# dmlc/difacto

Hardware: AMD Instinct MI355X
Metric: examples/sec (FM SGD worker step, Criteo-shape, V_dim=64) (higher is better)
Workload: dtype f32

## Files before the change

difacto_amd/capi.py:

```python
import ctypes as C
import os

import numpy as np

_HERE = os.path.dirname(os.path.abspath(__file__))
LIB_PATH = os.environ.get("DIFACTO_HIP_LIB") or os.path.join(_HERE, "libdifacto_hip.so")

FEA_COUNT, WEIGHT, GRADIENT = 1, 2, 3
INIT_REFRAND, INIT_HASH = 0, 1
U64MAX = 2 ** 64 - 1

SYMBOLS = [
    "dfh_last_error", "dfh_updater_param_default", "dfh_ctx_create", "dfh_ctx_destroy", "dfh_ctx_sync",
    "dfh_ctx_stream", "dfh_ctx_device", "dfh_reverse_bytes", "dfh_encode_fea_grp_id", "dfh_table_create",
    "dfh_table_destroy", "dfh_table_size", "dfh_table_param", "dfh_table_bytes", "dfh_pull", "dfh_push",
    "dfh_table_export", "dfh_table_import", "dfh_fm_predict", "dfh_fm_calcgrad", "dfh_loss_evaluate",
    "dfh_auc_times_n", "dfh_batch_create", "dfh_batch_destroy", "dfh_batch_load_host", "dfh_batch_load_device",
    "dfh_localize", "dfh_batch_load_localized_host", "dfh_batch_get_localized", "dfh_batch_shape", "dfh_sgd_step",
    "dfh_batch_progress", "dfh_batch_get_pred", "dfh_row_stride", "dfh_shard_pull", "dfh_shard_push_count",
    "dfh_shard_push_grad", "dfh_batch_forward", "dfh_batch_backward", "dfh_batch_device_keys", "dfh_malloc",
    "dfh_free", "dfh_memcpy_h2d", "dfh_memcpy_d2h", "dfh_ctx_set_timing", "dfh_ctx_get_timing", "dfh_kernel_name",
    "dfh_table_warm_start", "dfh_ctx_set_pipeline", "dfh_batch_lookup", "dfh_localize_lookup", "dfh_rowbuf_create", "dfh_rowbuf_destroy", "dfh_rowbuf_load_host", "dfh_batch_gather_rows", "dfh_batch_set_option", "dfh_batch_key_ranges", "dfh_batch_attach_device",
    "dfh_batch_key_ranges_device", "dfh_shard_resolve", "dfh_shard_pull_resolved", "dfh_shard_push_count_resolved",
    "dfh_shard_push_grad_resolved", "dfh_table_check", "dfh_ctx_set_timing_mask", "dfh_table_save", "dfh_table_load", "dfh_shard_resolve_multi", "dfh_shard_push_count_multi",
    "dfh_shard_push_grad_multi", "dfh_shard_count_pull_multi", "dfh_shard_push_grad_listed", "dfh_shard_release", "dfh_ctx_set_option", "dfh_table_set_has_aux", "dfh_table_has_aux",
    "dfh_comm_unique_id", "dfh_comm_create_rccl", "dfh_comm_create_callback", "dfh_comm_destroy", "dfh_comm_rank", "dfh_comm_world",
    "dfh_comm_allreduce_sum", "dfh_shard_create", "dfh_shard_destroy", "dfh_shard_owned_range", "dfh_shard_step", "dfh_shard_prefetch_counts",
    "dfh_shard_pull_host", "dfh_shard_push_host", "dfh_comm_allgather", "dfh_shard_balanced_splits", "dfh_shard_set_exchange", "dfh_shard_set_timing", "dfh_shard_get_timing",
    "dfh_comm_stats", "dfh_comm_info", "dfh_comm_selfcheck", "dfh_comm_wire_probe", "dfh_table_capacity", "dfh_batch_prepare_rows", "dfh_rowbuf_load_host_slices",
    "dfh_rowbuf_set_labels", "dfh_batch_prepare_cached", "dfh_batch_get_rows",
    "dfh_batch_create_many", "dfh_shard_multi_words", "dfh_shard_reserve", "dfh_comm_create_loopback", "dfh_comm_loopback_feed", "dfh_comm_loopback_wire", "dfh_comm_loopback_wire_time",
    "dfh_vec_inner_multi", "dfh_vec_combine", "dfh_vec_line_step", "dfh_lbfgs_create", "dfh_lbfgs_destroy", "dfh_lbfgs_add_chunk",
    "dfh_lbfgs_init_model", "dfh_lbfgs_shape", "dfh_lbfgs_get_model", "dfh_lbfgs_set_weights", "dfh_lbfgs_calc_grad",
    "dfh_lbfgs_prepare_direction", "dfh_lbfgs_calc_direction", "dfh_lbfgs_line_search", "dfh_lbfgs_evaluate", "dfh_lbfgs_create_sharded",
    "dfh_lbfgs_owned_range", "dfh_lbfgs_set_model", "dfh_lbfgs_get_vector", "dfh_bcd_set_model",
    "dfh_bcd_create", "dfh_bcd_destroy", "dfh_bcd_add_chunk", "dfh_bcd_build", "dfh_bcd_shape", "dfh_bcd_block_info",
    "dfh_bcd_epoch", "dfh_bcd_step", "dfh_bcd_get_model", "dfh_bcd_get_pred", "dfh_batch_split_entries",
    "dfh_bcd_create_sharded",
    "dfh_textchunk_create", "dfh_textchunk_destroy", "dfh_textchunk_parse_criteo", "dfh_textchunk_rows", "dfh_textchunk_ids",
    "dfh_rowbuf_load_slices",
]
XCHG_COUNTS, XCHG_KEYS, XCHG_CNT, XCHG_ROWS, XCHG_GRADS, XCHG_OTHER = range(6)
SHARD_STAGES = ("counts", "L", "K", "R", "RW", "F", "G", "P")
K_COUNT = 8
K_LOCALIZE, K_LOOKUP, K_FORWARD, K_BACKWARD, K_PULL, K_PUSH, K_MISC, K_AUC = range(8)


class UpdaterParam(C.Structure):
    _fields_ = [("l1", C.c_float), ("l2", C.c_float), ("V_l2", C.c_float), ("lr", C.c_float),
                ("lr_beta", C.c_float), ("V_lr", C.c_float), ("V_lr_beta", C.c_float),
                ("V_init_scale", C.c_float), ("V_dim", C.c_int), ("V_threshold", C.c_int),
                ("seed", C.c_uint), ("init_mode", C.c_int)]


class Progress(C.Structure):
    _fields_ = [("loss", C.c_float), ("penalty", C.c_float), ("auc", C.c_float),
                ("nnz_w", C.c_float), ("nrows", C.c_float)]


class Slice(C.Structure):
# ... 40 lines not shown
    L.dfh_reverse_bytes.restype = u64
    L.dfh_reverse_bytes.argtypes = [u64]
    L.dfh_encode_fea_grp_id.restype = u64
    L.dfh_encode_fea_grp_id.argtypes = [u64, i32, i32]
    L.dfh_table_create.argtypes = [vp, PP(UpdaterParam), u64, PP(vp)]
    L.dfh_table_destroy.argtypes = [vp]
    L.dfh_table_size.argtypes = [vp, PP(u64)]
    L.dfh_table_param.argtypes = [vp, PP(UpdaterParam)]
    L.dfh_table_capacity.argtypes = [vp, PP(u64), PP(u64)]
    L.dfh_table_bytes.restype = u64
    L.dfh_table_bytes.argtypes = [vp]
    L.dfh_pull.argtypes = [vp, vp, sz, vp, PP(sz), vp, PP(sz)]
    L.dfh_push.argtypes = [vp, vp, sz, i32, vp, sz, vp, sz]
    L.dfh_table_export.argtypes = [vp, u64, vp, vp, vp, vp, PP(u64)]
    L.dfh_table_import.argtypes = [vp, u64, vp, vp, vp, vp]
    L.dfh_fm_predict.argtypes = [vp, i32, sz, vp, vp, vp, vp, sz, vp, vp, sz, vp]
    L.dfh_fm_calcgrad.argtypes = [vp, i32, sz, vp, vp, vp, vp, vp, sz, vp, vp, sz, vp, vp]
    L.dfh_loss_evaluate.argtypes = [vp, vp, vp, sz, PP(f32)]
    L.dfh_auc_times_n.argtypes = [vp, vp, vp, sz, PP(f32)]
    L.dfh_batch_create.argtypes = [vp, sz, sz, PP(vp)]
    L.dfh_batch_destroy.argtypes = [vp]
    L.dfh_batch_create_many.argtypes = [vp, i32, sz, sz, PP(vp)]
    L.dfh_batch_split_entries.argtypes = [vp, vp]
    L.dfh_batch_load_host.argtypes = [vp, sz, vp, vp, vp, vp]
    L.dfh_batch_load_device.argtypes = [vp, sz, sz, vp, vp, vp, vp]
    L.dfh_batch_attach_device.argtypes = [vp, sz, sz, vp, vp, vp, vp]
    L.dfh_localize.argtypes = [vp, u64]
    L.dfh_batch_load_localized_host.argtypes = [vp, sz, vp, vp, vp, vp, vp, vp, sz]
    L.dfh_batch_get_localized.argtypes = [vp, PP(sz), vp, vp, vp]
    L.dfh_batch_shape.argtypes = [vp, PP(sz), PP(sz), PP(sz)]
    L.dfh_sgd_step.argtypes = [vp, vp, i32, i32]
    L.dfh_batch_progress.argtypes = [vp, PP(Progress), i32]
    L.dfh_batch_get_pred.argtypes = [vp, vp]
    L.dfh_row_stride.restype = sz
    L.dfh_row_stride.argtypes = [i32]
    L.dfh_shard_pull.argtypes = [vp, vp, sz, vp]
    L.dfh_shard_push_count.argtypes = [vp, vp, sz, vp]
    L.dfh_shard_push_grad.argtypes = [vp, vp, sz, vp]
    L.dfh_batch_forward.argtypes = [vp, i32, vp]
    L.dfh_batch_backward.argtypes = [vp, i32, vp, vp]
    L.dfh_batch_device_keys.argtypes = [vp, PP(vp), PP(vp), PP(sz)]
    L.dfh_malloc.argtypes = [vp, sz, PP(vp)]
    L.dfh_free.argtypes = [vp, vp]
    L.dfh_memcpy_h2d.argtypes = [vp, vp, vp, sz]
    L.dfh_memcpy_d2h.argtypes = [vp, vp, vp, sz]
    L.dfh_table_warm_start.argtypes = [vp, vp, sz, f32, f32]
# ... 539 lines not shown
        lab = np.zeros(nrows, np.float32)
        _ck(lib().dfh_batch_get_rows(self.h, _p(off), _p(lab)))
        return off, lab

    def sgd_step(self, table, is_train=True, push_cnt=False):
        _ck(lib().dfh_sgd_step(table.h, self.h, 1 if is_train else 0, 1 if push_cnt else 0))

    def progress(self, reset=True):
        p = Progress()
        _ck(lib().dfh_batch_progress(self.h, C.byref(p), 1 if reset else 0))
        return p

    def pred(self):
        nrows, _, _ = self.shape(want_U=False)
        out = np.zeros(nrows, np.float32)
        _ck(lib().dfh_batch_get_pred(self.h, _p(out)))
        return out

    def split_entries(self):
        n = C.c_uint32(0)
        _ck(lib().dfh_batch_split_entries(self.h, C.byref(n)))
        return int(n.value)

    def forward(self, V_dim, d_rows):
        _ck(lib().dfh_batch_forward(self.h, V_dim, _dp(d_rows)))

    def backward(self, V_dim, d_rows, d_grads):
        _ck(lib().dfh_batch_backward(self.h, V_dim, _dp(d_rows), _dp(d_grads)))

    def key_ranges(self, nparts):
        out = np.zeros(nparts + 1, np.uint32)
        _ck(lib().dfh_batch_key_ranges(self.h, nparts, _p(out)))
        return out

    def device_keys(self):
        a, b, u = C.c_void_p(), C.c_void_p(), C.c_size_t(0)
        _ck(lib().dfh_batch_device_keys(self.h, C.byref(a), C.byref(b), C.byref(u)))
        return a.value, b.value, u.value

    def device_key_ptrs(self):
        a, b = C.c_void_p(), C.c_void_p()
        _ck(lib().dfh_batch_device_keys(self.h, C.byref(a), C.byref(b), None))
        return a.value, b.value

    def key_ranges_device(self, nparts, d_bounds, d_splits=None):
        _ck(lib().dfh_batch_key_ranges_device(self.h, nparts, _dp(d_splits), _dp(d_bounds)))
# ... 385 lines not shown
```

difacto_amd/csrc/dfh_api.hip:

```cpp
#include <algorithm>
#include <chrono>
#include <cstring>
#include <mutex>
#include <new>
#include <thread>

#include <hip/hip_ext.h>
#include <rocprim/rocprim.hpp>

#include "dfh_kernels.hip"
#include "dfh_localize.hip"
#include "dfh_update.hip"
#include "dfh_riders.hip"

using namespace dfh;

namespace dfh {
static thread_local std::string g_err;
void set_error(const std::string& msg) { g_err = msg; }
}

struct dfh_ctx {
  int device = 0;
  hipStream_t stream = nullptr;
// ... 2435 lines not shown
    v.bkeys = b->d_keys;
    v.bpos = b->d_bpos;
    v.skeys = b->d_skeys;
    v.spos = b->d_spos;
    v.first_key = b->d_first_key;
    v.last_key = b->d_last_key;
    v.nheads = b->d_nheads;
    v.lh = b->d_lh;
    EmitOut& o = b->loc_o;
    o.value = b->has_value ? b->d_value : (const float*)nullptr;
    o.feaids = b->d_feaids;
    o.col_ptr = b->d_col_ptr;
    o.index = b->d_index;
    o.s_row = b->d_s_row;
    o.s_val = b->d_s_val;
    o.d_U = b->d_U;
    o.sl.mid = b->d_mid;
    o.sl.mid_ent = b->d_mid_ent;
    o.sl.hot = b->d_hot;
    o.sl.hot_ent = b->d_hot_ent;
    o.sl.few = b->d_few;
    o.sl.few_ent = b->d_few_ent;
    v.split_n = b->d_U + 2;
    b->loc_big = big;
#ifndef DFH_LOC_GRID_CAP
#define DFH_LOC_GRID_CAP 1024
#endif
    b->loc_gsort = (unsigned)std::min<int>(P, big ? LOC_BIG_BUCKETS : DFH_LOC_GRID_CAP);
    if (cold && P > 1) {
      const uint32_t S = (uint32_t)P * LOC_OVERSAMPLE;
      const uint32_t nt = (S + 255) / 256;
      hipLaunchKernelGGL(k_ss_sample, dim3(nt), dim3(256), 0, s, v);
      hipLaunchKernelGGL(k_ss_rank, dim3(nt * nt), dim3(256), 0, s, v);
      hipLaunchKernelGGL(k_loc_splitters, dim3(nt), dim3(256), 0, s, v);
    }
    if (c->single_queue && !cold && !big && !probe) {
      b->pend_stage = 0;
      c->pend.push_back(b);
    } else {
      for (int st = 0; st < RID_STAGES; ++st) {
        launch_loc_stage(b, st, s, probe);
        if (st == RID_COUNT && b->loc_fuse_gather) {
          int rcg = gather_queued(b, s);
          b->loc_fuse_gather = false;
          if (rcg) return rcg;
        }
      }
    }
    b->spl_P = P;
    b->seg_nb = (uint32_t)P;
  } else {
    hipLaunchKernelGGL(k_rdx_keys, dim3(g), dim3(256), 0, s, b->d_raw, N, max_index, b->d_keys, b->d_pos);
    size_t tb = b->temp_bytes;
    DFH_HIP(rocprim::radix_sort_pairs(b->d_temp, tb, b->d_keys, b->d_skeys, b->d_pos, b->d_spos, (size_t)N, 0, 64, s));
    hipLaunchKernelGGL(k_rdx_heads, dim3(g), dim3(256), 0, s, b->d_skeys, N, b->d_head);
    tb = b->temp_bytes;
    DFH_HIP(rocprim::inclusive_scan(b->d_temp, tb, b->d_head, b->d_uid, (size_t)N, rocprim::plus<uint32_t>(), s));
    hipLaunchKernelGGL(k_rdx_emit, dim3(g), dim3(256), 0, s, b->d_skeys, b->d_spos, b->d_head, b->d_uid, N, (uint32_t)b->nrows,
                       b->d_offset, b->has_value ? b->d_value : (const float*)nullptr, b->d_feaids, b->d_col_ptr, b->d_index,
                       b->d_s_row, b->d_s_val, b->d_U);
    hipLaunchKernelGGL(k_seg_lists_reset, dim3(1), dim3(64), 0, s, b->d_mid, b->d_hot, b->d_few, b->d_U + 2);
    hipLaunchKernelGGL(k_seg_lists, dim3((unsigned)std::max<size_t>(1, std::min<size_t>((N + 1023) / 1024, 256))), dim3(1024), 0, s,
                       b->d_col_ptr, b->d_U, b->d_mid, b->d_hot, b->d_few, b->d_mid_ent, b->d_hot_ent, b->d_few_ent);
    b->seg_nb = 1;
    if (probe)
      hipLaunchKernelGGL(k_lookup, dim3(grid_for_threads(b->nnz, c)), dim3(256), 0, s, probe->v, b->d_feaids, b->d_U, 0u, b->d_urow,
                         (const float*)nullptr, b->d_col_ptr, 0, (uint32_t*)nullptr, 0, (uint2*)nullptr, AucFin{nullptr, 0u, nullptr});
  }
  delete tsp;
  DFH_HIP(hipGetLastError());
  b->localized = true;
  b->has_cnt = false;
  if (probe) b->looked_up = probe;
  return prep_end(b);
// ... 263 lines not shown
  }
  rc = step_math(t, b, is_train, push_cnt, kAllKeys, nullptr, x, [&](bool) -> int {
    if (is_train && refrand) DFH_HIP(hipMemsetAsync(b->d_need, 0, (size_t)Nb * 4, s));
    return DFH_OK;
  });
  if (rc) return rc;
  if (is_train && refrand) {
    rc = refrand_flush(t, b->d_feaids, b->d_U, Nb, b->d_urow, b->d_need, b->d_rank, b->d_total);
    if (rc) return rc;
  }
  return main_end(b);
}

int dfh_batch_split_entries(dfh_batch* b, uint32_t* n) {
  DFH_ARG(b && n, "dfh_batch_split_entries: NULL argument");
  dfh_ctx* c = b->ctx;
  DFH_HIP(hipSetDevice(c->device));
  if (b->pend_stage < RID_STAGES) {
    int rc = flush_pending(b);
    if (rc) return rc;
  }
  if (b->ready_pending) DFH_HIP(hipStreamWaitEvent(c->stream, b->ev_ready, 0));
  DFH_HIP(hipMemcpyAsync(n, b->d_U + 2 + b->split_last, sizeof(uint32_t), hipMemcpyDeviceToHost, c->stream));
  DFH_HIP(hipStreamSynchronize(c->stream));
  return DFH_OK;
}

int dfh_batch_forward(dfh_batch* b, int V_dim, const float* d_rows) {
  DFH_ARG(b && b->localized && d_rows, "dfh_batch_forward: bad argument");
  const int kp = (V_dim + 3) / 4 * 4;
  int rc = ensure_xv(b, kp);
  if (rc) return rc;
  b->nrows_seen += (float)b->nrows;
  rc = main_begin(b);
  if (rc) return rc;
  rc = launch_forward(b, packed_src(d_rows, V_dim), V_dim, kp);
  if (rc) return rc;
  return main_end(b);
}

int dfh_batch_backward(dfh_batch* b, int V_dim, const float* d_rows, float* d_grads) {
  DFH_ARG(b && b->localized && d_rows && d_grads, "dfh_batch_backward: bad argument");
  const int kp = (V_dim + 3) / 4 * 4;
  if (b->nnz == 0) return DFH_OK;
  TableView dummy{};
  int rc = launch_backward<false>(b, packed_src(d_rows, V_dim), dummy, d_grads, dfh_row_stride(V_dim), V_dim, kp, nullptr);
// ... 93 lines not shown
```

difacto_amd/csrc/dfh_localize.hip:

```cpp
#ifndef DFH_LOCALIZE_HIP_
#define DFH_LOCALIZE_HIP_
#include "dfh_internal.h"
#include "dfh_feed_layout.h"

namespace dfh {

constexpr int LOC_OVERSAMPLE = 8;
constexpr int LOC_MAX_BUCKETS = 1024;
constexpr int LOC_BIG_BUCKETS = 4096;
constexpr int LOC_AVG_BUCKET = 384;
constexpr int LOC_MIN_AVG = 48;
constexpr int LOC_MAX_AVG = 700;
constexpr int LOC_LDS_CAP = 1024;
#ifndef DFH_LOC_TILE_THREADS
#define DFH_LOC_TILE_THREADS 1024
#endif
constexpr int LOC_TILE_THREADS = DFH_LOC_TILE_THREADS;
constexpr int LOC_PER_THREAD = LOC_TILE / LOC_TILE_THREADS;
constexpr int LOC_SORT_THREADS = 256;
constexpr int LOC_EMIT_THREADS = 256;

struct LocView {
  const uint64_t* raw;
  uint32_t n;
// ... 3 lines not shown
  int ntiles;
  int force_global;
  int tb;
  uint32_t nrows;
  const uint32_t* offset;
  const uint32_t* rowid;
  uint64_t* smp_key;
  uint32_t* smp_pos;
  uint32_t* smp_rank;
  uint64_t* spl_key;
  uint32_t* spl_pos;
  uint32_t* packed;
  uint32_t* run_off;
  uint32_t* btotal;
  uint32_t* bstart;
  uint64_t* bkeys;
  uint32_t* bpos;
  uint64_t* skeys;
  uint32_t* spos;
  uint64_t* first_key;
  uint64_t* last_key;
  uint32_t* nheads;
  uint32_t* lh;
  uint32_t* split_n;
};

struct SegListsOut {
  uint2* mid;
  SegEnt* mid_ent;
  uint2* hot;
  SegEnt* hot_ent;
  uint2* few;
  SegEnt* few_ent;
};

__device__ __forceinline__ uint64_t make_key(uint64_t id, uint64_t max_index) {
  const uint64_t m = (max_index == ~0ULL) ? (id == ~0ULL ? 0ULL : id) : id % max_index;
  return reverse_bytes(m);
}

constexpr int LOC_XCDS = 8;

__device__ __forceinline__ bool comp_less(uint64_t ka, uint32_t pa, uint64_t kb, uint32_t pb) {
  return ka < kb || (ka == kb && pa < pb);
}

// ... 96 lines not shown
  const float* src_val[LOC_GATHER_SEGS];
  const uint32_t* h_rows;
  const uint32_t* h_off;
  const float* h_lab;
  const uint32_t* h_tile_row;
  uint64_t* dst_raw;
  float* dst_val;
  uint32_t* dst_off;
  float* dst_lab;
};
constexpr size_t loc_gather_smem() { return (size_t)(LOC_GATHER_ROWS + 1) * 4 + 4 + (size_t)LOC_GATHER_ROWS * 8; }
template <typename T>
__device__ __forceinline__ T loc_sel(const T (&a)[LOC_GATHER_SEGS], uint32_t sg) {
  T r = a[0];
#pragma unroll
  for (int x = 1; x < LOC_GATHER_SEGS; ++x) r = sg == (uint32_t)x ? a[x] : r;
  return r;
}

template <int MAXB>
constexpr size_t loc_count_smem() { return (size_t)MAXB * 16; }
template <int MAXB, int THREADS>
constexpr size_t loc_scatter_smem() { return (size_t)MAXB * 4 + (THREADS / 64) * 4; }
constexpr size_t loc_sort_smem() { return (size_t)LOC_LDS_CAP * 24 + 2 * (LOC_SORT_THREADS / 64) * 4; }
constexpr size_t loc_emit_smem() { return (2 * (LOC_EMIT_THREADS / 64) + 4) * 4; }

template <int MAXB, int THREADS, bool GATHER = false>
__device__ __forceinline__ void loc_count_block(const LocView& v, const uint32_t bid, const uint32_t nblk, char* smem,
                                                const GatherSrc* gp = nullptr) {
  constexpr int PER = LOC_TILE / THREADS;
  static_assert(PER * THREADS == LOC_TILE, "a tile is a whole number of elements per thread");
  uint64_t* sk = reinterpret_cast<uint64_t*>(smem);
  uint32_t* sp = reinterpret_cast<uint32_t*>(smem + (size_t)MAXB * 8);
  uint32_t* hist = sp + MAXB;
  const int P = v.P;
  for (int b = threadIdx.x; b < P; b += THREADS) {
    hist[b] = 0;
    sk[b] = b < P - 1 ? v.spl_key[b] : ~0ULL;
    sp[b] = b < P - 1 ? v.spl_pos[b] : ~0u;
  }
  const uint32_t base = bid * LOC_TILE;
  if (bid == 0 && threadIdx.x == 0 && v.split_n) *v.split_n = 0u;
  uint64_t key[PER];
  if (GATHER) {
    const GatherSrc& g = *gp;
    uint32_t* roff = reinterpret_cast<uint32_t*>(smem + loc_count_smem<MAXB>());
    uint64_t* rsrc = reinterpret_cast<uint64_t*>(roff + LOC_GATHER_ROWS + 2);
    const uint32_t row0 = g.h_tile_row[bid], row1 = g.h_tile_row[bid + 1];
    const uint32_t nr = min(row1, v.nrows - 1u) - row0 + 1u;
    for (uint32_t q = threadIdx.x; q <= nr; q += THREADS) roff[q] = g.h_off[row0 + q];
    for (uint32_t q = threadIdx.x; q < nr; q += THREADS) {
      const uint32_t r = row0 + q;
      uint32_t sg = 0;
#pragma unroll
      for (int x = 1; x < LOC_GATHER_SEGS; ++x) sg += (x < g.nseg && r >= g.seg_row0[x]) ? 1u : 0u;
      rsrc[q] = ((uint64_t)loc_sel(g.src_off, sg)[g.h_rows[r]] << 2) | sg;
    }
    __syncthreads();
#pragma unroll
    for (int e = 0; e < PER; ++e) {
      const uint32_t i = base + e * THREADS + threadIdx.x;
      key[e] = ~0ULL;
      if (i < v.n) {
        uint32_t lo = 0, hi = nr - 1u;
// ... 158 lines not shown

template <int MAXB>
__global__ void __launch_bounds__(LOC_TILE_THREADS) k_loc_scatter(LocView v) {
  __shared__ __attribute__((aligned(16))) char smem[loc_scatter_smem<MAXB, LOC_TILE_THREADS>()];
  loc_scatter_block<MAXB, LOC_TILE_THREADS>(v, blockIdx.x, smem);
}

template <int J>
__device__ __forceinline__ uint32_t loc_net_partner(uint32_t x) {
  static_assert(J == 1 || J == 2 || J == 4 || J == 8, "DPP reaches the partners inside a row of 16 lanes");
  if constexpr (J == 1) return (uint32_t)__builtin_amdgcn_mov_dpp((int)x, 0xB1, 0xf, 0xf, false);
  if constexpr (J == 2) return (uint32_t)__builtin_amdgcn_mov_dpp((int)x, 0x4E, 0xf, 0xf, false);
  if constexpr (J == 4) {
    const int y = __builtin_amdgcn_mov_dpp((int)x, 0x141, 0xf, 0xf, false);
    return (uint32_t)__builtin_amdgcn_mov_dpp(y, 0x1B, 0xf, 0xf, false);
  }
  return (uint32_t)__builtin_amdgcn_mov_dpp((int)x, 0x128, 0xf, 0xf, false);
}
constexpr uint64_t loc_net_keeps_max(int K, int J) {
  uint64_t m = 0;
  for (int i = 0; i < 64; ++i) m |= (uint64_t)(((i & J) != 0) != ((i & K) != 0)) << i;
  return m;
}
template <int K, int J>
__device__ __forceinline__ void loc_net_stage(uint32_t& klo, uint32_t& khi, uint32_t& tag) {
  uint32_t mlo, mhi;
  asm volatile("s_mov_b32 %0, %2\n\ts_mov_b32 %1, %3"
               : "=s"(mlo), "=s"(mhi)
               : "i"((int32_t)(uint32_t)loc_net_keeps_max(K, J)), "i"((int32_t)(uint32_t)(loc_net_keeps_max(K, J) >> 32)));
  const uint64_t mask = ((uint64_t)mhi << 32) | mlo;
  const bool keeps_max = __builtin_amdgcn_inverse_ballot_w64(mask);
  if constexpr (J >= 16) {
    uint32_t alo, ahi, at, blo, bhi, bt;
#define DFH_NET_SWAP(a, b, x)                                                                                       \
    {                                                                                                                 \
      const auto r = J == 16 ? __builtin_amdgcn_permlane16_swap(x, x, false, false) : __builtin_amdgcn_permlane32_swap(x, x, false, false); \
      a = r[0];                                                                                                       \
      b = r[1];                                                                                                       \
    }
    DFH_NET_SWAP(alo, blo, klo)
    DFH_NET_SWAP(ahi, bhi, khi)
    DFH_NET_SWAP(at, bt, tag)
#undef DFH_NET_SWAP
    const bool out_of_order = comp_less(((uint64_t)bhi << 32) | blo, bt, ((uint64_t)ahi << 32) | alo, at);
    const bool take_b = out_of_order != keeps_max;
    klo = take_b ? blo : alo;
    khi = take_b ? bhi : ahi;
    tag = take_b ? bt : at;
  } else {
    const uint32_t olo = loc_net_partner<J>(klo), ohi = loc_net_partner<J>(khi), ot = loc_net_partner<J>(tag);
    const bool partner_less = comp_less(((uint64_t)ohi << 32) | olo, ot, ((uint64_t)khi << 32) | klo, tag);
    const bool take = partner_less != keeps_max;
    klo = take ? olo : klo;
    khi = take ? ohi : khi;
    tag = take ? ot : tag;
  }
}
template <int K, int J>
__device__ __forceinline__ void loc_net_merge(uint32_t& klo, uint32_t& khi, uint32_t& tag) {
  loc_net_stage<K, J>(klo, khi, tag);
  if constexpr (J > 1) loc_net_merge<K, J / 2>(klo, khi, tag);
}
template <int K = 2>
__device__ __forceinline__ void loc_net_sort64(uint32_t& klo, uint32_t& khi, uint32_t& tag) {
  loc_net_merge<K, K / 2>(klo, khi, tag);
  if constexpr (K < 64) loc_net_sort64<K * 2>(klo, khi, tag);
}

__device__ __forceinline__ bool loc_sort_bucket_lds(const LocView& v, uint32_t beg, uint32_t n, uint64_t* ak, uint32_t* ap,
                                                    uint64_t* bk, uint32_t* bp) {
  const uint64_t* gk = v.bkeys + beg;
  const uint32_t* gp = v.bpos + beg;
  uint64_t* sk = bk;
  uint32_t* sp = bp;
  const uint32_t lane = threadIdx.x & 63;
  for (uint32_t c0 = (threadIdx.x >> 6) * 64; c0 < n; c0 += LOC_SORT_THREADS) {
    const uint32_t idx = c0 + lane;
    const bool valid = idx < n;
    const uint64_t mk = valid ? gk[idx] : ~0ULL;
    uint32_t klo = (uint32_t)mk, khi = (uint32_t)(mk >> 32);
    uint32_t mp = valid ? gp[idx] : ~0u;
    loc_net_sort64(klo, khi, mp);
    if (valid) {
      bk[idx] = ((uint64_t)khi << 32) | klo;
      bp[idx] = mp;
    }
  }
  __syncthreads();
  constexpr int E = LOC_LDS_CAP / LOC_SORT_THREADS;
  constexpr int G = 2;
  static_assert(E * LOC_SORT_THREADS == LOC_LDS_CAP && E % G == 0 && LOC_SORT_THREADS % 64 == 0,
                "a thread carries E elements of a full bucket, G at a time");
  uint64_t* dk = ak;
  uint32_t* dp = ap;
  uint32_t sh = 6;
  for (uint32_t L = 64; L < n; L <<= 1, ++sh) {
    for (int g = 0; g < E && g * LOC_SORT_THREADS < (int)n; g += G) {
      uint64_t mk[G];
      uint32_t mp[G], at[G], end[G];
#pragma unroll
      for (int e = 0; e < G; ++e) {
        const uint32_t idx = threadIdx.x + (g + e) * LOC_SORT_THREADS;
        const bool valid = idx < n;
        const uint32_t sib = ((idx >> sh) ^ 1u) << sh;
        mk[e] = valid ? sk[idx] : 0ULL;
// ... 1 lines not shown
        at[e] = min(sib, n);
        end[e] = valid ? min(sib + L, n) : at[e];
      }
      for (uint32_t step = L; step; step >>= 1) {
        uint64_t ok[G];
        uint32_t op[G];
#pragma unroll
        for (int e = 0; e < G; ++e) {
          const uint32_t q = at[e] + step <= end[e] ? at[e] + step - 1u : 0u;
          ok[e] = sk[q];
          op[e] = sp[q];
        }
#pragma unroll
        for (int e = 0; e < G; ++e)
          if (at[e] + step <= end[e] && comp_less(ok[e], op[e], mk[e], mp[e])) at[e] += step;
      }
#pragma unroll
      for (int e = 0; e < G; ++e) {
        const uint32_t idx = threadIdx.x + (g + e) * LOC_SORT_THREADS;
        if (idx < n) {
          const uint32_t dst = idx + at[e] - min((idx & ~(L - 1u)) | L, n);
          dk[dst] = mk[e];
          dp[dst] = mp[e];
        }
      }
    }
    __syncthreads();
    uint64_t* tk = sk; sk = dk; dk = tk;
    uint32_t* tp = sp; sp = dp; dp = tp;
  }
  return sk == ak;
}
__device__ __forceinline__ void loc_sort_bucket_global(const LocView& v, uint32_t beg, uint32_t n) {
  uint64_t* xk = v.bkeys + beg;
  uint32_t* xp = v.bpos + beg;
  uint64_t* yk = v.skeys + beg;
  uint32_t* yp = v.spos + beg;
  const uint32_t lane = threadIdx.x & 63;
  for (uint32_t c0 = (threadIdx.x >> 6) * 64; c0 < n; c0 += LOC_SORT_THREADS) {
    const uint32_t idx = c0 + lane;
    const bool valid = idx < n;
    const uint64_t mk = valid ? xk[idx] : ~0ULL;
    const uint32_t mp = valid ? xp[idx] : ~0u;
    const uint32_t lim = min(64u, n - c0);
    uint32_t rank = 0;
    for (uint32_t j = 0; j < lim; ++j) rank += comp_less(xk[c0 + j], xp[c0 + j], mk, mp) ? 1u : 0u;
// ... 58 lines not shown
  }
  cnt = (uint32_t)__builtin_amdgcn_readlane((int)wave_inclusive<false>(cnt), 63);
  last = (uint32_t)__builtin_amdgcn_readlane((int)wave_inclusive<true>(last), 63);
  if ((threadIdx.x & 63) == 0) {
    red[0][threadIdx.x >> 6] = cnt;
    red[1][threadIdx.x >> 6] = last;
  }
  __syncthreads();
  BucketSummary r;
  r.nheads = 1;
  r.lh = 0;
  r.first_key = 0;
  r.last_key = 0;
  if (threadIdx.x == 0) {
    for (int w = 0; w < LOC_SORT_THREADS / 64; ++w) {
      r.nheads += red[0][w];
      r.lh = max(r.lh, red[1][w]);
    }
    r.first_key = sk[0];
    r.last_key = sk[n - 1];
  }
  return r;
}

__device__ __forceinline__ void loc_sort_block(const LocView& v, const uint32_t bid, const uint32_t nblk, char* smem) {
  uint64_t* ak = reinterpret_cast<uint64_t*>(smem);
  uint64_t* bk = ak + LOC_LDS_CAP;
  uint32_t* ap = reinterpret_cast<uint32_t*>(bk + LOC_LDS_CAP);
  uint32_t* bp = ap + LOC_LDS_CAP;
  uint32_t (*red)[LOC_SORT_THREADS / 64] = reinterpret_cast<uint32_t (*)[LOC_SORT_THREADS / 64]>(bp + LOC_LDS_CAP);
  for (uint32_t b = bid; b < (uint32_t)v.P; b += nblk) {
    __syncthreads();
    const uint32_t beg = v.bstart[b], end = v.bstart[b + 1];
    const uint32_t n = end - beg;
    if (threadIdx.x < LOC_XCDS) v.btotal[threadIdx.x * v.bstride + b] = 0;
    if (n == 0) {
      if (threadIdx.x == 0) {
        v.nheads[b] = 0;
        v.lh[b] = 0;
        v.first_key[b] = 0;
        v.last_key[b] = 0;
      }
      continue;
    }
    BucketSummary sm;
    if (n <= LOC_LDS_CAP && !v.force_global) {
      const bool in_a = loc_sort_bucket_lds(v, beg, n, ak, ap, bk, bp);
      sm = loc_bucket_summary<true>(in_a ? ak : bk, in_a ? ap : bp, n, v.skeys + beg, v.spos + beg, red);
    } else {
      loc_sort_bucket_global(v, beg, n);
      sm = loc_bucket_summary<false>(v.skeys + beg, v.spos + beg, n, nullptr, nullptr, red);
    }
    if (threadIdx.x == 0) {
      v.nheads[b] = sm.nheads;
      v.lh[b] = sm.lh;
      v.first_key[b] = sm.first_key;
      v.last_key[b] = sm.last_key;
    }
  }
}
__global__ void __launch_bounds__(LOC_SORT_THREADS) k_loc_sort(LocView v) {
  extern __shared__ __attribute__((aligned(16))) char smem[];
  loc_sort_block(v, blockIdx.x, gridDim.x, smem);
}

template <int NW, bool PROBE>
__device__ __forceinline__ void loc_emit_bucket(const LocView& v, uint32_t b, uint32_t beg, uint32_t n, const uint64_t* sk,
                                                const uint32_t* sp, uint32_t cont, uint32_t ubase, uint32_t carry1,
                                                const float* __restrict__ value,
                                                uint64_t* __restrict__ feaids, uint32_t* __restrict__ col_ptr,
                                                uint32_t* __restrict__ index, uint32_t* __restrict__ s_row,
// ... 157 lines not shown
```

include/difacto_hip.h:

```cpp
#ifndef DIFACTO_HIP_H_
#define DIFACTO_HIP_H_
#include <stddef.h>
#include <stdint.h>

#ifdef __cplusplus
extern "C" {
#endif

enum {
  DFH_OK = 0,
  DFH_ERR_ARG = 1,
  DFH_ERR_HIP = 2,
  DFH_ERR_CAPACITY = 3,
  DFH_ERR_STATE = 4
};

enum { DFH_FEA_COUNT = 1, DFH_WEIGHT = 2, DFH_GRADIENT = 3 };

enum {
  DFH_INIT_REFRAND = 0,
  DFH_INIT_HASH = 1
};

typedef struct {
// ... 107 lines not shown
  size_t first;
  size_t nnz;
} dfh_slice;
int dfh_rowbuf_load_slices(dfh_rowbuf* rb, size_t nrows, const size_t* offset, int nslices, const dfh_slice* slices);
int dfh_batch_gather_rows(dfh_batch* b, size_t nrows, const size_t* offset, const float* label, int nseg, dfh_rowbuf* const* bufs,
                          const uint32_t* const* rows, const size_t* seg_rows);
int dfh_batch_prepare_rows(dfh_table* t, dfh_batch* b, size_t nrows, const size_t* offset, const float* label, int nseg,
                           dfh_rowbuf* const* bufs, const uint32_t* const* rows, const size_t* seg_rows, uint64_t max_index);
int dfh_rowbuf_set_labels(dfh_rowbuf* rb, size_t nrows, const float* label);
int dfh_batch_prepare_cached(dfh_table* t, dfh_batch* b, size_t nrows, int nseg, dfh_rowbuf* const* bufs, const uint32_t* const* rows,
                             const size_t* seg_rows, uint64_t max_index);

int dfh_batch_load_localized_host(dfh_batch* b, size_t nrows, const size_t* offset, const uint32_t* index,
                                  const float* value, const float* label, const uint64_t* feaids,
                                  const float* feacnt, size_t U);
int dfh_batch_get_localized(dfh_batch* b, size_t* U, uint64_t* feaids, float* feacnt, uint32_t* index);
int dfh_batch_shape(dfh_batch* b, size_t* nrows, size_t* nnz, size_t* U);
int dfh_batch_get_rows(dfh_batch* b, uint32_t* offset, float* label);

int dfh_sgd_step(dfh_table* t, dfh_batch* b, int is_train, int push_cnt);
int dfh_batch_progress(dfh_batch* b, dfh_progress* out, int reset);
int dfh_batch_get_pred(dfh_batch* b, float* pred);
int dfh_batch_split_entries(dfh_batch* b, uint32_t* n);

size_t dfh_row_stride(int V_dim);
int dfh_shard_pull(dfh_table* t, const uint64_t* d_keys, size_t n, float* d_rows);
int dfh_shard_push_count(dfh_table* t, const uint64_t* d_keys, size_t n, const float* d_cnt);
int dfh_shard_push_grad(dfh_table* t, const uint64_t* d_keys, size_t n, const float* d_grads);
int dfh_batch_forward(dfh_batch* b, int V_dim, const float* d_rows);
int dfh_batch_backward(dfh_batch* b, int V_dim, const float* d_rows, float* d_grads);
int dfh_batch_device_keys(dfh_batch* b, const uint64_t** d_feaids, const float** d_feacnt, size_t* U);
int dfh_batch_key_ranges(dfh_batch* b, int nparts, uint32_t* bounds);
int dfh_batch_key_ranges_device(dfh_batch* b, int nparts, const uint64_t* d_splits, int64_t* d_bounds);

int dfh_shard_resolve(dfh_table* t, const uint64_t* d_keys, size_t n, uint32_t* d_rowid);
int dfh_shard_pull_resolved(dfh_table* t, const uint32_t* d_rowid, size_t n, float* d_rows);
int dfh_shard_push_count_resolved(dfh_table* t, const uint32_t* d_rowid, const uint64_t* d_keys, size_t n, const float* d_cnt);
int dfh_shard_push_grad_resolved(dfh_table* t, const uint32_t* d_rowid, const uint64_t* d_keys, size_t n, const float* d_grads);
size_t dfh_shard_multi_words(size_t n, int nsrc);
int dfh_shard_resolve_multi(dfh_table* t, const uint64_t* d_keys, const size_t* seg, int nsrc, int mask_slot,
                            uint32_t* d_rowid);
int dfh_shard_push_count_multi(dfh_table* t, const uint32_t* d_rowid, const uint64_t* d_keys, const size_t* seg, int nsrc,
                               int mask_slot, const float* d_cnt);
int dfh_shard_push_grad_multi(dfh_table* t, const uint32_t* d_rowid, const uint64_t* d_keys, const size_t* seg, int nsrc,
                              int mask_slot, const float* d_grads);
int dfh_shard_count_pull_multi(dfh_table* t, uint32_t* d_rowid, const uint64_t* d_keys, const size_t* seg, int nsrc, int mask_slot,
// ... 97 lines not shown
```

Before: 88.50 million.

## Sort localize buckets on packed offset words with exact-resort fallback

The LDS bucket sort now subtracts the bucket's minimum key and packs the key offset together with part of the position tag into a single 64-bit word. The bitonic network and merge-path steps can then compare plain words instead of doing a two-field (key, pos) comparison, and merge ranks come from a binary search over the packed words. A summary pass unpacks keys and tags and checks for cases where the packing could lose ordering (overflow or tag collisions), and falls back to the original exact sort when that happens. A device counter and an API entry report how many buckets needed the resort. This adds complexity and a redo path in exchange for cheaper comparisons in the localize sort.

New measurement: 89.32 million, median of 6. No clear change (+0.9%).

```diff
diff --git a/difacto_amd/capi.py b/difacto_amd/capi.py
--- a/difacto_amd/capi.py
+++ b/difacto_amd/capi.py
@@ -35,7 +35,7 @@
     "dfh_lbfgs_prepare_direction", "dfh_lbfgs_calc_direction", "dfh_lbfgs_line_search", "dfh_lbfgs_evaluate", "dfh_lbfgs_create_sharded",
     "dfh_lbfgs_owned_range", "dfh_lbfgs_set_model", "dfh_lbfgs_get_vector", "dfh_bcd_set_model",
     "dfh_bcd_create", "dfh_bcd_destroy", "dfh_bcd_add_chunk", "dfh_bcd_build", "dfh_bcd_shape", "dfh_bcd_block_info",
-    "dfh_bcd_epoch", "dfh_bcd_step", "dfh_bcd_get_model", "dfh_bcd_get_pred", "dfh_batch_split_entries",
+    "dfh_bcd_epoch", "dfh_bcd_step", "dfh_bcd_get_model", "dfh_bcd_get_pred", "dfh_batch_split_entries", "dfh_batch_resorted_buckets",
     "dfh_bcd_create_sharded",
     "dfh_textchunk_create", "dfh_textchunk_destroy", "dfh_textchunk_parse_criteo", "dfh_textchunk_rows", "dfh_textchunk_ids",
     "dfh_rowbuf_load_slices",
@@ -122,6 +122,7 @@
     L.dfh_batch_destroy.argtypes = [vp]
     L.dfh_batch_create_many.argtypes = [vp, i32, sz, sz, PP(vp)]
     L.dfh_batch_split_entries.argtypes = [vp, vp]
+    L.dfh_batch_resorted_buckets.argtypes = [vp, vp]
     L.dfh_batch_load_host.argtypes = [vp, sz, vp, vp, vp, vp]
     L.dfh_batch_load_device.argtypes = [vp, sz, sz, vp, vp, vp, vp]
     L.dfh_batch_attach_device.argtypes = [vp, sz, sz, vp, vp, vp, vp]
@@ -707,6 +708,11 @@
         _ck(lib().dfh_batch_split_entries(self.h, C.byref(n)))
         return int(n.value)
 
+    def resorted_buckets(self):
+        n = C.c_uint32(0)
+        _ck(lib().dfh_batch_resorted_buckets(self.h, C.byref(n)))
+        return int(n.value)
+
     def forward(self, V_dim, d_rows):
         _ck(lib().dfh_batch_forward(self.h, V_dim, _dp(d_rows)))
 
diff --git a/difacto_amd/csrc/dfh_api.hip b/difacto_amd/csrc/dfh_api.hip
--- a/difacto_amd/csrc/dfh_api.hip
+++ b/difacto_amd/csrc/dfh_api.hip
@@ -2481,6 +2481,7 @@
     o.sl.few = b->d_few;
     o.sl.few_ent = b->d_few_ent;
     v.split_n = b->d_U + 2;
+    v.resort_n = b->d_U + 4;
     b->loc_big = big;
 #ifndef DFH_LOC_GRID_CAP
 #define DFH_LOC_GRID_CAP 1024
@@ -2509,6 +2510,7 @@
     b->spl_P = P;
     b->seg_nb = (uint32_t)P;
   } else {
+    DFH_HIP(hipMemsetAsync(b->d_U + 4, 0, sizeof(uint32_t), s));
     hipLaunchKernelGGL(k_rdx_keys, dim3(g), dim3(256), 0, s, b->d_raw, N, max_index, b->d_keys, b->d_pos);
     size_t tb = b->temp_bytes;
     DFH_HIP(rocprim::radix_sort_pairs(b->d_temp, tb, b->d_keys, b->d_skeys, b->d_pos, b->d_spos, (size_t)N, 0, 64, s));
@@ -2818,6 +2820,20 @@
   }
   if (b->ready_pending) DFH_HIP(hipStreamWaitEvent(c->stream, b->ev_ready, 0));
   DFH_HIP(hipMemcpyAsync(n, b->d_U + 2 + b->split_last, sizeof(uint32_t), hipMemcpyDeviceToHost, c->stream));
+  DFH_HIP(hipStreamSynchronize(c->stream));
+  return DFH_OK;
+}
+
+int dfh_batch_resorted_buckets(dfh_batch* b, uint32_t* n) {
+  DFH_ARG(b && n, "dfh_batch_resorted_buckets: NULL argument");
+  dfh_ctx* c = b->ctx;
+  DFH_HIP(hipSetDevice(c->device));
+  if (b->pend_stage < RID_STAGES) {
+    int rc = flush_pending(b);
+    if (rc) return rc;
+  }
+  if (b->ready_pending) DFH_HIP(hipStreamWaitEvent(c->stream, b->ev_ready, 0));
+  DFH_HIP(hipMemcpyAsync(n, b->d_U + 4, sizeof(uint32_t), hipMemcpyDeviceToHost, c->stream));
   DFH_HIP(hipStreamSynchronize(c->stream));
   return DFH_OK;
 }
diff --git a/difacto_amd/csrc/dfh_localize.hip b/difacto_amd/csrc/dfh_localize.hip
--- a/difacto_amd/csrc/dfh_localize.hip
+++ b/difacto_amd/csrc/dfh_localize.hip
@@ -49,6 +49,7 @@
   uint64_t* last_key;
   uint32_t* nheads;
   uint32_t* lh;
+  uint32_t* resort_n;
   uint32_t* split_n;
 };
 
@@ -191,7 +192,7 @@
 constexpr size_t loc_count_smem() { return (size_t)MAXB * 16; }
 template <int MAXB, int THREADS>
 constexpr size_t loc_scatter_smem() { return (size_t)MAXB * 4 + (THREADS / 64) * 4; }
-constexpr size_t loc_sort_smem() { return (size_t)LOC_LDS_CAP * 24 + 2 * (LOC_SORT_THREADS / 64) * 4; }
+constexpr size_t loc_sort_smem() { return (size_t)LOC_LDS_CAP * 24 + 3 * (LOC_SORT_THREADS / 64) * 4 + (LOC_SORT_THREADS / 64) * 8 + 8; }
 constexpr size_t loc_emit_smem() { return (2 * (LOC_EMIT_THREADS / 64) + 4) * 4; }
 
 template <int MAXB, int THREADS, bool GATHER = false>
@@ -209,6 +210,7 @@
     sp[b] = b < P - 1 ? v.spl_pos[b] : ~0u;
   }
   const uint32_t base = bid * LOC_TILE;
+  if (bid == 0 && threadIdx.x == 0 && v.resort_n) *v.resort_n = 0u;
   if (bid == 0 && threadIdx.x == 0 && v.split_n) *v.split_n = 0u;
   uint64_t key[PER];
   if (GATHER) {
@@ -413,7 +415,12 @@
   for (int i = 0; i < 64; ++i) m |= (uint64_t)(((i & J) != 0) != ((i & K) != 0)) << i;
   return m;
 }
-template <int K, int J>
+template <bool WORD>
+__device__ __forceinline__ bool loc_net_less(uint64_t ka, uint32_t pa, uint64_t kb, uint32_t pb) {
+  if constexpr (WORD) return ka < kb;
+  return comp_less(ka, pa, kb, pb);
+}
+template <bool WORD, int K, int J>
 __device__ __forceinline__ void loc_net_stage(uint32_t& klo, uint32_t& khi, uint32_t& tag) {
   uint32_t mlo, mhi;
   asm volatile("s_mov_b32 %0, %2\n\ts_mov_b32 %1, %3"
@@ -433,33 +440,33 @@
     DFH_NET_SWAP(ahi, bhi, khi)
     DFH_NET_SWAP(at, bt, tag)
 #undef DFH_NET_SWAP
-    const bool out_of_order = comp_less(((uint64_t)bhi << 32) | blo, bt, ((uint64_t)ahi << 32) | alo, at);
+    const bool out_of_order = loc_net_less<WORD>(((uint64_t)bhi << 32) | blo, bt, ((uint64_t)ahi << 32) | alo, at);
     const bool take_b = out_of_order != keeps_max;
     klo = take_b ? blo : alo;
     khi = take_b ? bhi : ahi;
     tag = take_b ? bt : at;
   } else {
     const uint32_t olo = loc_net_partner<J>(klo), ohi = loc_net_partner<J>(khi), ot = loc_net_partner<J>(tag);
-    const bool partner_less = comp_less(((uint64_t)ohi << 32) | olo, ot, ((uint64_t)khi << 32) | klo, tag);
+    const bool partner_less = loc_net_less<WORD>(((uint64_t)ohi << 32) | olo, ot, ((uint64_t)khi << 32) | klo, tag);
     const bool take = partner_less != keeps_max;
     klo = take ? olo : klo;
     khi = take ? ohi : khi;
     tag = take ? ot : tag;
   }
 }
-template <int K, int J>
+template <bool WORD, int K, int J>
 __device__ __forceinline__ void loc_net_merge(uint32_t& klo, uint32_t& khi, uint32_t& tag) {
-  loc_net_stage<K, J>(klo, khi, tag);
-  if constexpr (J > 1) loc_net_merge<K, J / 2>(klo, khi, tag);
-}
-template <int K = 2>
+  loc_net_stage<WORD, K, J>(klo, khi, tag);
+  if constexpr (J > 1) loc_net_merge<WORD, K, J / 2>(klo, khi, tag);
+}
+template <bool WORD, int K = 2>
 __device__ __forceinline__ void loc_net_sort64(uint32_t& klo, uint32_t& khi, uint32_t& tag) {
-  loc_net_merge<K, K / 2>(klo, khi, tag);
-  if constexpr (K < 64) loc_net_sort64<K * 2>(klo, khi, tag);
-}
-
-__device__ __forceinline__ bool loc_sort_bucket_lds(const LocView& v, uint32_t beg, uint32_t n, uint64_t* ak, uint32_t* ap,
-                                                    uint64_t* bk, uint32_t* bp) {
+  loc_net_merge<WORD, K, K / 2>(klo, khi, tag);
+  if constexpr (K < 64) loc_net_sort64<WORD, K * 2>(klo, khi, tag);
+}
+
+__device__ __forceinline__ bool loc_sort_bucket_lds_exact(const LocView& v, uint32_t beg, uint32_t n, uint64_t* ak, uint32_t* ap,
+                                                          uint64_t* bk, uint32_t* bp) {
   const uint64_t* gk = v.bkeys + beg;
   const uint32_t* gp = v.bpos + beg;
   uint64_t* sk = bk;
@@ -471,7 +478,7 @@
     const uint64_t mk = valid ? gk[idx] : ~0ULL;
     uint32_t klo = (uint32_t)mk, khi = (uint32_t)(mk >> 32);
     uint32_t mp = valid ? gp[idx] : ~0u;
-    loc_net_sort64(klo, khi, mp);
+    loc_net_sort64<false>(klo, khi, mp);
     if (valid) {
       bk[idx] = ((uint64_t)khi << 32) | klo;
       bp[idx] = mp;
@@ -519,6 +526,146 @@
           const uint32_t dst = idx + at[e] - min((idx & ~(L - 1u)) | L, n);
           dk[dst] = mk[e];
           dp[dst] = mp[e];
+        }
+      }
+    }
+    __syncthreads();
+    uint64_t* tk = sk; sk = dk; dk = tk;
+    uint32_t* tp = sp; sp = dp; dp = tp;
+  }
+  return sk == ak;
+}
+
+struct LocWordFmt {
+  uint32_t tb;
+  uint32_t pm;
+  uint32_t tm;
+  __device__ __forceinline__ explicit LocWordFmt(int tb_) : tb((uint32_t)tb_), pm(0xFFFFFFFFu >> tb_), tm((1u << tb_) - 1u) {}
+  __device__ __forceinline__ uint64_t key(uint64_t lo, uint64_t a, uint32_t w) const { return lo + ((a & ~(uint64_t)pm) | (uint64_t)(w >> tb)); }
+  __device__ __forceinline__ uint32_t tag(uint64_t a, uint32_t w) const { return (((uint32_t)a & pm) << tb) | (w & tm); }
+};
+__device__ __forceinline__ uint64_t wave_min_u64(uint64_t x) {
+#define DFH_DPP_STEP(ctrl, row_mask)                                                                                      \
+  {                                                                                                                       \
+    const uint32_t ylo = (uint32_t)__builtin_amdgcn_update_dpp(-1, (int)(uint32_t)x, ctrl, row_mask, 0xf, false);         \
+    const uint32_t yhi = (uint32_t)__builtin_amdgcn_update_dpp(-1, (int)(uint32_t)(x >> 32), ctrl, row_mask, 0xf, false); \
+    const uint64_t y = ((uint64_t)yhi << 32) | ylo;                                                                       \
+    x = y < x ? y : x;                                                                                                    \
+  }
+  DFH_DPP_STEP(0x111, 0xf)
+  DFH_DPP_STEP(0x112, 0xf)
+  DFH_DPP_STEP(0x114, 0xf)
+  DFH_DPP_STEP(0x118, 0xf)
+  DFH_DPP_STEP(0x142, 0xa)
+  DFH_DPP_STEP(0x143, 0xc)
+#undef DFH_DPP_STEP
+  return ((uint64_t)(uint32_t)__builtin_amdgcn_readlane((int)(uint32_t)(x >> 32), 63) << 32) |
+         (uint32_t)__builtin_amdgcn_readlane((int)(uint32_t)x, 63);
+}
+__device__ __forceinline__ bool loc_sort_bucket_lds(const LocView& v, uint32_t beg, uint32_t n, uint64_t* ak, uint32_t* ap,
+                                                    uint64_t* bk, uint32_t* bp, uint64_t* wmin ,
+                                                    uint32_t* over , uint64_t* lo_out) {
+  const uint64_t* gk = v.bkeys + beg;
+  const uint32_t* gp = v.bpos + beg;
+  const LocWordFmt f(v.tb);
+#define DFH_OPAQUE_TID(t) uint32_t t = threadIdx.x; asm volatile("" : "+v"(t));
+  uint64_t lo = ~0ULL;
+  DFH_OPAQUE_TID(t1)
+  {
+    constexpr int E = LOC_LDS_CAP / LOC_SORT_THREADS;
+    uint64_t k[E];
+    uint32_t p[E];
+#pragma unroll
+    for (int e = 0; e < E; ++e) {
+      const uint32_t idx = t1 + e * LOC_SORT_THREADS;
+      k[e] = gk[min(idx, n - 1u)];
+      p[e] = gp[min(idx, n - 1u)];
+    }
+#pragma unroll
+    for (int e = 0; e < E; ++e) {
+      const uint32_t idx = t1 + e * LOC_SORT_THREADS;
+      if (idx < n) {
+        bk[idx] = k[e];
+        bp[idx] = p[e];
+      }
+      lo = k[e] < lo ? k[e] : lo;
+    }
+  }
+  lo = wave_min_u64(lo);
+  if ((t1 & 63) == 0) wmin[t1 >> 6] = lo;
+  if (t1 == 0) *over = 0u;
+  __syncthreads();
+#pragma unroll
+  for (int w = 0; w < LOC_SORT_THREADS / 64; ++w) lo = wmin[w] < lo ? wmin[w] : lo;
+  lo = ((uint64_t)(uint32_t)__builtin_amdgcn_readfirstlane((int)(uint32_t)(lo >> 32)) << 32) |
+       (uint32_t)__builtin_amdgcn_readfirstlane((int)(uint32_t)lo);
+  *lo_out = lo;
+  uint64_t* sk = bk;
+  uint32_t* sp = bp;
+  const uint32_t np = n <= 64u ? 64u : 1u << (32 - __builtin_clz(n - 1u));
+  DFH_OPAQUE_TID(t2)
+  const uint32_t lane = t2 & 63;
+  for (uint32_t c0 = (uint32_t)__builtin_amdgcn_readfirstlane((int)(t2 >> 6)) * 64; c0 < np; c0 += LOC_SORT_THREADS) {
+    const uint32_t idx = c0 + lane;
+    const bool valid = idx < n;
+    const uint64_t off = (valid ? bk[idx] : 0ULL) - lo;
+    const uint32_t tag = valid ? bp[idx] : 0u;
+    uint32_t alo = valid ? (((uint32_t)off & ~f.pm) | (tag >> f.tb)) : (0xFFFFFC00u | idx);
+    uint32_t ahi = valid ? (uint32_t)(off >> 32) : ~0u;
+    uint32_t mw = (((uint32_t)off & f.pm) << f.tb) | (tag & f.tm);
+    if (c0 < n) {
+      if (__builtin_amdgcn_ballot_w64(valid && ahi == ~0u && alo >= 0xFFFFFC00u) != 0) *over = 1u;
+      loc_net_sort64<true>(alo, ahi, mw);
+    }
+    bk[idx] = ((uint64_t)ahi << 32) | alo;
+    bp[idx] = mw;
+  }
+  __syncthreads();
+  constexpr int E = LOC_LDS_CAP / LOC_SORT_THREADS;
+  constexpr int G = 2;
+  static_assert(E * LOC_SORT_THREADS == LOC_LDS_CAP && E % G == 0 && LOC_SORT_THREADS % 64 == 0,
+                "a thread carries E elements of a full bucket, G at a time");
+  uint64_t* dk = ak;
+  uint32_t* dp = ap;
+  uint32_t sh = 6;
+  DFH_OPAQUE_TID(t3)
+#undef DFH_OPAQUE_TID
+  for (uint32_t L = 64; L < np; L <<= 1, ++sh) {
+    for (int g = 0; g < E && g * LOC_SORT_THREADS < (int)np; g += G) {
+      uint64_t ma[G];
+      uint32_t mw[G];
+      const uint64_t* pa[G];
+#pragma unroll
+      for (int e = 0; e < G; ++e) {
+        const uint32_t idx = t3 + (g + e) * LOC_SORT_THREADS;
+        const bool valid = idx < np;
+        ma[e] = valid ? sk[idx] : 0ULL;
+        mw[e] = valid ? sp[idx] : 0u;
+        pa[e] = sk + (valid ? ((idx >> sh) ^ 1u) << sh : 0u) - 1;
+      }
+      for (uint32_t s = L; s; s >>= 1) {
+        const uint32_t step = s > 1u ? s >> 1 : 1u;
+        const uint64_t* q[G];
+        uint64_t oa[G];
+#pragma unroll
+        for (int e = 0; e < G; ++e) {
+          q[e] = pa[e] + step;
+          oa[e] = *q[e];
+        }
+        static_assert(G == 2, "the line below names the G words");
+        asm volatile("" : "+v"(oa[0]), "+v"(oa[1]));
+#pragma unroll
+        for (int e = 0; e < G; ++e) pa[e] = oa[e] < ma[e] ? q[e] : pa[e];
+      }
+#pragma unroll
+      for (int e = 0; e < G; ++e) {
+        const uint32_t idx = t3 + (g + e) * LOC_SORT_THREADS;
+        if (idx < np) {
+          const uint32_t sib = ((idx >> sh) ^ 1u) << sh;
+          const uint32_t cnt = ((uint32_t)(uintptr_t)pa[e] + 8u - (uint32_t)(uintptr_t)(sk + sib)) >> 3;
+          const uint32_t dst = (idx & ~(2u * L - 1u)) + (idx & (L - 1u)) + cnt;
+          dk[dst] = ma[e];
+          dp[dst] = mw[e];
         }
       }
     }
@@ -623,6 +770,57 @@
   }
   return r;
 }
+__device__ __forceinline__ BucketSummary loc_bucket_summary_word(const uint64_t* sa, const uint32_t* sw, uint32_t n, uint64_t lo,
+                                                                 const LocWordFmt f, uint64_t* ok, uint32_t* op,
+                                                                 uint32_t (*red)[LOC_SORT_THREADS / 64], const uint32_t* over,
+                                                                 bool* redo) {
+  uint32_t cnt = 0, last = 0;
+  bool bad = false;
+  uint32_t t0 = threadIdx.x;
+  asm volatile("" : "+v"(t0));
+  for (uint32_t t = t0; t < n; t += LOC_SORT_THREADS) {
+    const uint64_t a = sa[t];
+    const uint32_t w = sw[t];
+    ok[t] = f.key(lo, a, w);
+    op[t] = f.tag(a, w);
+    if (t + 1 < n) {
+      const bool high_differs = ((a ^ sa[t + 1]) & ~(uint64_t)f.pm) != 0;
+      const bool low_differs = ((w ^ sw[t + 1]) >> f.tb) != 0;
+      if (high_differs || low_differs) {
+        ++cnt;
+        last = t + 1;
+      }
+      bad = bad || (!high_differs && low_differs);
+    }
+  }
+  cnt = (uint32_t)__builtin_amdgcn_readlane((int)wave_inclusive<false>(cnt), 63);
+  last = (uint32_t)__builtin_amdgcn_readlane((int)wave_inclusive<true>(last), 63);
+  const bool wave_bad = __builtin_amdgcn_ballot_w64(bad) != 0;
+  if ((threadIdx.x & 63) == 0) {
+    red[0][threadIdx.x >> 6] = cnt;
+    red[1][threadIdx.x >> 6] = last;
+    red[2][threadIdx.x >> 6] = wave_bad ? 1u : 0u;
+  }
+  __syncthreads();
+  BucketSummary r;
+  r.nheads = 1;
+  r.lh = 0;
+  r.first_key = 0;
+  r.last_key = 0;
+  uint32_t any_bad = *over;
+#pragma unroll
+  for (int w = 0; w < LOC_SORT_THREADS / 64; ++w) any_bad |= red[2][w];
+  *redo = __builtin_amdgcn_readfirstlane((int)any_bad) != 0;
+  if (threadIdx.x == 0) {
+    for (int w = 0; w < LOC_SORT_THREADS / 64; ++w) {
+      r.nheads += red[0][w];
+      r.lh = max(r.lh, red[1][w]);
+    }
+    r.first_key = f.key(lo, sa[0], sw[0]);
+    r.last_key = f.key(lo, sa[n - 1], sw[n - 1]);
+  }
+  return r;
+}
 
 __device__ __forceinline__ void loc_sort_block(const LocView& v, const uint32_t bid, const uint32_t nblk, char* smem) {
   uint64_t* ak = reinterpret_cast<uint64_t*>(smem);
@@ -630,6 +828,8 @@
   uint32_t* ap = reinterpret_cast<uint32_t*>(bk + LOC_LDS_CAP);
   uint32_t* bp = ap + LOC_LDS_CAP;
   uint32_t (*red)[LOC_SORT_THREADS / 64] = reinterpret_cast<uint32_t (*)[LOC_SORT_THREADS / 64]>(bp + LOC_LDS_CAP);
+  uint64_t* wmin = reinterpret_cast<uint64_t*>(red + 3);
+  uint32_t* over = reinterpret_cast<uint32_t*>(wmin + LOC_SORT_THREADS / 64);
   for (uint32_t b = bid; b < (uint32_t)v.P; b += nblk) {
     __syncthreads();
     const uint32_t beg = v.bstart[b], end = v.bstart[b + 1];
@@ -646,8 +846,16 @@
     }
     BucketSummary sm;
     if (n <= LOC_LDS_CAP && !v.force_global) {
-      const bool in_a = loc_sort_bucket_lds(v, beg, n, ak, ap, bk, bp);
-      sm = loc_bucket_summary<true>(in_a ? ak : bk, in_a ? ap : bp, n, v.skeys + beg, v.spos + beg, red);
+      uint64_t lo;
+      bool in_a = loc_sort_bucket_lds(v, beg, n, ak, ap, bk, bp, wmin, over, &lo);
+      bool redo;
+      sm = loc_bucket_summary_word(in_a ? ak : bk, in_a ? ap : bp, n, lo, LocWordFmt(v.tb), v.skeys + beg, v.spos + beg, red, over, &redo);
+      if (redo) {
+        __syncthreads();
+        in_a = loc_sort_bucket_lds_exact(v, beg, n, ak, ap, bk, bp);
+        sm = loc_bucket_summary<true>(in_a ? ak : bk, in_a ? ap : bp, n, v.skeys + beg, v.spos + beg, red);
+        if (threadIdx.x == 0 && v.resort_n) atomicAdd(v.resort_n, 1u);
+      }
     } else {
       loc_sort_bucket_global(v, beg, n);
       sm = loc_bucket_summary<false>(v.skeys + beg, v.spos + beg, n, nullptr, nullptr, red);
diff --git a/include/difacto_hip.h b/include/difacto_hip.h
--- a/include/difacto_hip.h
+++ b/include/difacto_hip.h
@@ -153,6 +153,7 @@
 int dfh_batch_progress(dfh_batch* b, dfh_progress* out, int reset);
 int dfh_batch_get_pred(dfh_batch* b, float* pred);
 int dfh_batch_split_entries(dfh_batch* b, uint32_t* n);
+int dfh_batch_resorted_buckets(dfh_batch* b, uint32_t* n);
 
 size_t dfh_row_stride(int V_dim);
 int dfh_shard_pull(dfh_table* t, const uint64_t* d_keys, size_t n, float* d_rows);
```
